# Westlake-AGI-Lab/WorldForge

Hardware: AMD Instinct MI355X
Metric: denoising steps/sec (81f x 480p, Wan2.1-14B) (higher is better)
Workload: dtype bf16

## Files before the change

include/wf_hip.h:

```cpp
#ifndef WF_HIP_H_
#define WF_HIP_H_

#include <stddef.h>
#include <stdint.h>

#ifdef __cplusplus
extern "C" {
#endif

#define WF_OK 0
#define WF_EINVAL (-1)
#define WF_EHIP (-2)
#define WF_ENOTSUP (-3)

#define WF_F32 0
#define WF_BF16 1

int wf_version(void);
const char* wf_last_error(void);
int wf_device_info(int dev, int* n_cu, int* clock_khz, char* name, int name_len);


int wf_cfg_combine(const void* cond, const void* uncond, void* out, int dt, float g, size_t n, void* stream);

// ... 41 lines not shown

size_t wf_farneback_workspace_bytes(int C, int T, int h, int w);
int wf_farneback_flows(const void* x, int dt, float* flow, int C, int T, int h, int w, int quant_mode, void* ws, void* stream);


#define WF_EPI_BF16 0
#define WF_EPI_BF16_GELU 1
#define WF_EPI_F32 2
#define WF_EPI_RESID 3
#define WF_EPI_F32_ACC 4
int wf_gemm_bf16(const void* X, const void* W, const float* bias, void* out, const float* gate, int M, int N, int K, int ldx,
                 int ldw, int ldo, int epilogue, void* stream);
int wf_gemm_bf16_batched(const void* X, const void* W, void* out, int batch, int M, int N, int K, int ldx, int ldw, int ldo,
                         int64_t bsx, int64_t bsw, int64_t bso, int epilogue, void* stream);
int wf_gemm_f16(const void* X, const void* W, const float* bias, void* out, int M, int N, int K, int ldx, int ldw, int ldo, int epilogue,
                float acc_scale, void* stream);
int wf_gemm_f16_batched(const void* X, const void* W, void* out, int batch, int M, int N, int K, int ldx, int ldw, int ldo, int64_t bsx,
                        int64_t bsw, int64_t bso, int epilogue, void* stream);
int wf_mx_quant_e4m3(const void* X, void* Q, void* S, int M, int K, int ldx, void* stream);
int wf_gemm_mxfp8(const void* Xq, const void* Xs, const void* Wq, const void* Ws, const float* bias, void* out, const float* gate, int M, int N,
                  int K, int ldx, int ldw, int ldo, int epilogue, void* stream);
int wf_lora_fold(const void* base, void* out, int N, int K, int n_adapters, const void* U0, const void* D0, int rank0, int nsep0,
                 float scale0, const void* U1, const void* D1, int rank1, int nsep1, float scale1, const void* U2, const void* D2,
                 int rank2, int nsep2, float scale2, const void* U3, const void* D3, int rank3, int nsep3, float scale3, void* stream);

int wf_attn_fwd(const void* Q, const void* K, const void* Vt, void* O, int H, int Lq, int Lkp, int kv_len, int seg_len,
                size_t seg_stride_bytes, int ldo, float softmax_scale, int accumulate, const float* kmax2, int kmax_n, int kmax_stride,
                const float* qmax2, int qmax_n, void* stream);
int wf_head_max_norm2(const void* X, int H, int L, int Lp, float* out, void* stream);
size_t wf_attn_split_workspace_bytes(int H, int Lq, int nsplit);
int wf_attn_cross2_fwd(const void* Q, const void* K, const void* Vt, void* O, int H, int Lq, int Lk1p, int kv_len1, int Lk2p, int kv_len2,
                       int ldo, float softmax_scale, void* stream);
int wf_attn_debug_body_counter(void* counters2);
int wf_attn_fwd_split(const void* Q, const void* K, const void* Vt, void* O, int H, int Lq, int Lkp, int kv_len, int seg_len,
                      size_t seg_stride_bytes, int ldo, float softmax_scale, int accumulate, int nsplit, void* workspace, const float* kmax2,
                      int kmax_n, int kmax_stride, const float* qmax2, int qmax_n, void* stream);
int wf_attn_fwd_part(const void* Q, const void* K, const void* Vt, int H, int Lq, int Lkp, int kv_len, int seg_len, size_t seg_stride_bytes,
                     int t_begin, int t_end, int t_begin2, int t_end2, int inner_splits, int part, int nparts, void* workspace, void* O_merge,
                     int ldo, const float* kmax2, int kmax_n, int kmax_stride, const float* qmax2, int qmax_n, void* stream);
int wf_attn_merge(void* O, int H, int Lq, int ldo, int accumulate, int nparts, const void* workspace, void* stream);

int wf_ln_modulate(const float* x, const float* mul, const float* add, void* out, int out_dtype, int L, int C, float eps,
                   int plus_one, void* stream);

int wf_rmsnorm_heads(const void* in, int ld, const float* weight, const float* cos_tab, const float* sin_tab, void* out, int L,
                     int Lout, int C, float eps, float out_scale, void* stream);
size_t wf_rmsnorm_heads_bound_ws_floats(int L, int C);
int wf_rmsnorm_heads_bound(const void* in, int ld, const float* weight, const float* cos_tab, const float* sin_tab, void* out, int L, int Lout,
                           int C, float eps, float out_scale, float* ws, float* max_norm2, void* stream);

int wf_v_transpose(const void* V, int ld, void* Vt, int L, int Lp, int H, void* stream);
int wf_v_transpose_seg(const void* V, int ld, void* Vt, int L, int Lp, int H, int head_stride_tiles, void* stream);
int wf_v_transpose_at(const void* V, int ld, void* Vt, int k0, int L, int Lp, int H, void* stream);

int wf_patchify(const void* x, void* tokens, int Cin, int T, int Hh, int Ww, void* stream);
int wf_unpatchify(const float* y, float* out, int Cout, int T, int Hh, int Ww, void* stream);

int wf_act(const void* a, int dt_a, const void* b, int dt_b, void* out, int dt_out, int mode, size_t n, void* stream);

int wf_lc_ln_modulate(const void* x, const float* mul, const float* add, int64_t mod_ld, int rows_per_group, int64_t row0,
                      const int* group_index, int plus_one, void* out, int L, int C, float eps, void* stream);
int wf_lc_gate_residual(void* x, const void* y, int64_t ldy, const float* gate, int64_t gate_ld, int rows_per_group, int64_t row0,
                        const int* group_index, int L, int C, void* stream);
int wf_lc_norm_heads(const void* in, int64_t ld, const float* weight, const float* cos_tab, const float* sin_tab, void* out, int L,
                     int Lout, int H, float eps, float out_scale, void* stream);
int wf_lc_swiglu(const void* in, int64_t ld, void* out, int L, int Hd, void* stream);
// ... 124 lines not shown
```

worldforge_amd/csrc/attention.hip:

```cpp
#include "common.h"
#include "mfma.h"

#include <climits>
#include <cstdlib>
#include <type_traits>
#include <utility>

using namespace wf;

namespace {

constexpr int D = 128;
constexpr int QB = 256;
constexpr int KB = 64;
constexpr int K_TILE_BYTES = KB * D * 2;
constexpr int V_TILE_BYTES = D * KB * 2;

struct AttnArgs {
  const uint16_t* Q;
  const uint16_t* K;
  const uint16_t* Vt;
  uint16_t* O;
  int H, Lq, Lkp, kv_len, ldo;
  int seg_len;
// ... 24 lines not shown
#define WF_ATTN_DMA_PLACE 0
#endif
#ifndef WF_ATTN_ABLATE
#define WF_ATTN_ABLATE 0
#endif
#ifdef WF_ATTN_TIMING
__device__ unsigned long long g_attn_cycles[32];
#endif

constexpr int MAX_MERGE = 11;
__device__ __forceinline__ float ws_at(const float (&w)[MAX_MERGE], int s) {
  float r = w[0];
#pragma unroll
  for (int i = 1; i < MAX_MERGE; ++i) r = s == i ? w[i] : r;
  return r;
}

__device__ __forceinline__ int swap23(int i) { return (i & ~12) | ((i & 4) << 1) | ((i & 8) >> 1); }


constexpr int NT4 = 256;

__device__ __forceinline__ float mul_rn(float a, float b) {
  float r;
  asm("v_mul_f32 %0, %1, %2" : "=v"(r) : "v"(a), "v"(b));
  return r;
}
__device__ __forceinline__ float add_rn(float a, float b) {
  float r;
  asm("v_add_f32 %0, %1, %2" : "=v"(r) : "v"(a), "v"(b));
  return r;
}

template <int KIND, bool NOMAX, bool PART = false>
__device__ __forceinline__ void attn_w4_body(const AttnArgs& a) {
  extern __shared__ __attribute__((aligned(16))) unsigned char smem[];
  constexpr int BUF_BYTES = K_TILE_BYTES + V_TILE_BYTES;
  constexpr int NBUF = 5;
  static_assert(NBUF * BUF_BYTES == 160 * 1024, "the ring is the whole LDS of a CU and the launch asks for exactly that (attn_launch: lds_w4)");
  static_assert((NT4 / 64) * 4 * 1024 == K_TILE_BYTES && (NT4 / 64) * 4 * 1024 == V_TILE_BYTES,
                "4 waves x (4 K + 4 V^T) pieces of 1 KiB (64 lanes x 16 B) cover a K tile and a V^T tile exactly: no piece may spill into the next ring slot");
  static_assert(K_TILE_BYTES % 1024 == 0 && BUF_BYTES % 16 == 0, "piece granularity / ds_read_b128 alignment of the slots");
  static_assert(NBUF >= 2 + 3, "ring too short for the 3-ahead staging with one barrier per two tiles");

  const int b = blockIdx.x;
  const int xcd = b & 7, j = b >> 3;
  const int hslot = j / a.n_qblk;
  const int head = hslot * 8 + xcd;
  const int qblk = j % a.n_qblk;
  if (head >= a.H) return;

  const int tid = threadIdx.x, lane = tid & 63, wid = tid >> 6;
  const int l31 = lane & 31, hi = lane >> 5;
  int q_row[2];
  bf16x8 qf[2][8];
#pragma unroll
  for (int x = 0; x < 2; ++x) {
    q_row[x] = qblk * QB + wid * 64 + x * 32 + l31;
    const uint16_t* qp = a.Q + ((size_t)head * a.Lq + min(q_row[x], a.Lq - 1)) * D;
#pragma unroll
    for (int st = 0; st < 8; ++st) qf[x][st] = as_bf16x8(*reinterpret_cast<const u32x4*>(qp + 16 * st + 8 * hi));
  }

  const int wu = __builtin_amdgcn_readfirstlane(wid);
  int ksrc[4], vsrc[4];
#pragma unroll
  for (int i = 0; i < 4; ++i) {
    const int piece = wu * 4 + i;
    const int kr = 4 * piece + (lane >> 4), ks = lane & 15;
    ksrc[i] = kr * D + ((ks ^ (kr & 15)) << 3);
    const int vr = 8 * piece + (lane >> 3), vs = lane & 7;
    vsrc[i] = vr * KB + ((vs ^ ((vr >> 1) & 7)) << 3);
  }
  const int tiles_per_seg = a.seg_len / KB;
  int krow_off[2], krow_sw[2];
#pragma unroll
  for (int kb = 0; kb < 2; ++kb) {
    int kr = kb * 32 + swap23(l31);
    krow_off[kb] = kr * 256;
    krow_sw[kb] = kr & 15;
  }
  int vrow_off[4], vrow_sw[4];
#pragma unroll
// ... 29 lines not shown
    const bool after = rel0 >= a.n_first;
    t_begin = after ? a.t_begin2 + (rel0 - a.n_first) : a.t_begin0 + rel0;
    ntiles_ = min(a.tiles_per_split, a.tiles_per_split2 - rel0);
    if (!after && rel0 + ntiles_ > a.n_first) {
      hole_at = a.n_first - rel0;
      hole_tiles = a.t_begin2 - a.t_end;
    }
  } else {
    t_begin = a.t_begin0 + (int)blockIdx.y * a.tiles_per_split;
    ntiles_ = min(a.tiles_per_split, min(ntiles_all, a.t_end) - t_begin);
  }
  const int* bsa = nullptr;
  const int tpe = (KIND == 3 && a.bsa_shift == 2) ? 2 : 1;
  const int mine = a.bsa_shift == 2 ? (wu >> 1) : wu;
  if constexpr (KIND == 3) {
    bsa = a.bsa_list + ((size_t)head * a.n_qblk + qblk) * a.bsa_max;
    ntiles_ = tpe * a.bsa_cnt[head * a.n_qblk + qblk];
    if (ntiles_ == 0) {
#pragma unroll
      for (int x = 0; x < 2; ++x)
        if (q_row[x] < a.Lq) {
          uint16_t* op = a.O + (size_t)q_row[x] * a.ldo + head * D;
          for (int d = hi * 64; d < hi * 64 + 64; d += 8) *reinterpret_cast<u32x4*>(op + d) = u32x4{0u, 0u, 0u, 0u};
        }
      return;
    }
  }
  const int ntiles = ntiles_;
  const bool ragged = KIND != 3 && KIND != 5 && (a.kv_len & (KB - 1)) != 0;
  const int rag_t = ragged ? ntiles_all - 2 - t_begin - hole_tiles : -1;
  const bool rag1 = KIND == 5 && (a.kv_len1 & (KB - 1)) != 0, rag2 = KIND == 5 && (a.kv_len & (KB - 1)) != 0;

  const size_t tile_bytes = (size_t)(KB * D * 2);
  const size_t seg_jump = a.seg_stride - (size_t)tiles_per_seg * tile_bytes;
  const size_t hole_bytes = (size_t)(hole_tiles / tiles_per_seg) * a.seg_stride;
  const int seg0 = t_begin / tiles_per_seg, in0 = t_begin - seg0 * tiles_per_seg;
  size_t st_off = (size_t)seg0 * a.seg_stride + ((size_t)head * tiles_per_seg + in0) * tile_bytes;
  int st_tile = 0, st_left = tiles_per_seg - in0;
  uint32_t st_base = wu * 4096;
  int e_stage = 0, e_mask = 0;
  int e_pref = 0, e_q[3] = {0, 0, 0};
  const int n_entries = KIND == 3 ? ntiles / tpe : 1;
  auto entry_index = [&](int tile) { return min(tpe == 2 ? (tile >> 1) : tile, n_entries - 1); };
  if constexpr (KIND == 3) {
    e_stage = __builtin_amdgcn_readfirstlane(bsa[0]);
    st_off = (size_t)(e_stage >> a.bsa_shift) * tpe * tile_bytes;
    e_q[0] = e_q[1] = e_q[2] = e_stage;
    e_pref = bsa[entry_index(1)];
  }
  auto stage_next = [&]() {
    ++st_tile;
    const bool live = st_tile < ntiles;
    if constexpr (KIND == 3) {
      if (live) {
        e_stage = __builtin_amdgcn_readfirstlane(e_pref);
        st_off = ((size_t)(e_stage >> a.bsa_shift) * tpe + (st_tile & (tpe - 1))) * tile_bytes;
      }
      e_pref = bsa[entry_index(st_tile + 1)];
      e_q[0] = e_q[1];
      e_q[1] = e_q[2];
      e_q[2] = e_stage;
      st_base = st_base + BUF_BYTES >= (uint32_t)(NBUF * BUF_BYTES) ? st_base + BUF_BYTES - NBUF * BUF_BYTES : st_base + BUF_BYTES;
      return;
    }
    const bool wrap = --st_left == 0;
    if constexpr (PART) {
      const bool hop = st_tile == hole_at;
      st_off += live ? (wrap ? tile_bytes + seg_jump + (hop ? hole_bytes : 0) : tile_bytes) : 0;
    } else {
      st_off += live ? (wrap ? tile_bytes + seg_jump : tile_bytes) : 0;
    }
    st_left = wrap ? tiles_per_seg : st_left;
    st_base = st_base + BUF_BYTES >= (uint32_t)(NBUF * BUF_BYTES) ? st_base + BUF_BYTES - NBUF * BUF_BYTES : st_base + BUF_BYTES;
  };
  const uint32_t smem_base = __builtin_amdgcn_readfirstlane(lds_offset(smem));
  uint32_t kbyte[4], vbyte[4];
#pragma unroll
  for (int i = 0; i < 4; ++i) {
    kbyte[i] = (uint32_t)ksrc[i] * 2u;
    vbyte[i] = (uint32_t)vsrc[i] * 2u;
  }
  auto stage_piece = [&](int i) {
    const unsigned char* kb_ = reinterpret_cast<const unsigned char*>(a.K) + st_off;
    const unsigned char* vb_ = reinterpret_cast<const unsigned char*>(a.Vt) + st_off;
    if (i < 4)
// ... 115 lines not shown
    for (int x = 0; x < 2; ++x)
#pragma unroll
      for (int kb = 0; kb < 2; ++kb)
#pragma unroll
        for (int r = 0; r < 16; ++r) {
          int key = tile_in_ctx * KB + 32 * kb + 16 * (r >> 3) + 8 * hi + (r & 7);
          if (key >= len) sb[B][x][kb][r] = -INFINITY;
        }
  };

  auto mask_unselected = [&](auto BC, int entry) {
    constexpr int B = decltype(BC)::value;
    if (!((entry >> mine) & 1)) {
#pragma unroll
      for (int x = 0; x < 2; ++x)
#pragma unroll
        for (int kb = 0; kb < 2; ++kb)
#pragma unroll
          for (int r = 0; r < 16; ++r) sb[B][x][kb][r] = -INFINITY;
    }
  };

#ifndef WF_ATTN_PF4
#define WF_ATTN_PF4 4
#endif
  constexpr int PF4 = WF_ATTN_PF4;
  u32x4 ring[PF4];
#if defined(WF_ATTN_TIMING) && WF_ATTN_TIMING != 2
  unsigned long long tacc[20] = {};
#define W4MARK(k) do { const unsigned long long n__ = __builtin_readcyclecounter(); tacc[k] += n__ - tlast; tlast = n__; } while (0)
#else
#define W4MARK(k) do { } while (0)
#endif
  auto tile = [&](auto BC, int t, int slot0) {
    constexpr int B = decltype(BC)::value;
    const int slot1 = slot0 + 1 == NBUF ? 0 : slot0 + 1;
    const int slot2 = slot1 + 1 == NBUF ? 0 : slot1 + 1;
    const unsigned char* sK1 = smem + slot1 * BUF_BYTES;
    const unsigned char* sV0 = smem + slot0 * BUF_BYTES + K_TILE_BYTES;
    const unsigned char* sK2 = smem + slot2 * BUF_BYTES;
    float tq_[64], pq[64];
    float ls[2][4];
    uint32_t pk[2][4] = {{0u, 0u, 0u, 0u}, {0u, 0u, 0u, 0u}};
    float mx[2][4];
    float mn[2] = {0.f, 0.f};
#if defined(WF_ATTN_TIMING) && WF_ATTN_TIMING != 2
    unsigned long long tlast = __builtin_readcyclecounter();
#endif
    __builtin_amdgcn_sched_barrier(0);
    for_const<64>([&](auto GC) {
      auto& sb_ = sb;
      auto& pf_ = pf;
      auto& o_ = o;
      auto& ring_ = ring;
      auto& tq__ = tq_;
      auto& pq_ = pq;
      auto& ls_ = ls;
      auto& pk_ = pk;
      auto& mx_ = mx;
      auto& mcq_ = mcq;
      constexpr int g = decltype(GC)::value;
      constexpr int q = g & 1;
      if constexpr (g < 32) {
        constexpr int i = g >> 1;
        mfma_s(sb_[1 - B][q][i & 1], ring_[i % PF4], qf[q][i >> 1], i < 2, PS ? &minit[q] : nullptr);
        __builtin_amdgcn_sched_barrier(0);
        if constexpr (q == 1 && !(WF_ATTN_ABLATE & 4)) {
// ... 64 lines not shown
          constexpr int kb = ch >> 1, r0 = (ch & 1) + 4 * st;
          if constexpr (st == 0) {
            asm volatile("v_max_f32 %0, %1, %2" : "=v"(mx_[x][ch]) : "v"(sb_[1 - B][x][kb][r0]), "v"(sb_[1 - B][x][kb][r0 + 2]));
          } else {
            asm volatile("v_max3_f32 %0, %0, %1, %2" : "+v"(mx_[x][ch]) : "v"(sb_[1 - B][x][kb][r0]), "v"(sb_[1 - B][x][kb][r0 + 2]));
          }
        });
      }
      if constexpr (!NOMAX && (g == 60 || g == 61)) {
        constexpr int x = g - 60;
        asm volatile("v_max3_f32 %0, %1, %2, %3" : "=v"(mn[x]) : "v"(mx_[x][0]), "v"(mx_[x][1]), "v"(mx_[x][2]));
        asm volatile("v_max_f32 %0, %0, %1" : "+v"(mn[x]) : "v"(mx_[x][3]));
      }
      if constexpr (!NOMAX && (g == 62 || g == 63)) {
        constexpr int x = g - 62;
        const unsigned mu = __float_as_uint(mn[x]);
        auto sw = __builtin_amdgcn_permlane32_swap(mu, mu, false, false);
        if constexpr (PS) {
          const float zero = 0.0f;
          asm volatile("v_max3_f32 %0, %1, %2, %3" : "=v"(mn[x]) : "v"(__uint_as_float(sw[0])), "v"(__uint_as_float(sw[1])), "v"(zero));
        } else {
          asm volatile("v_max3_f32 %0, %1, %2, %3" : "=v"(mn[x]) : "v"(__uint_as_float(sw[0])), "v"(__uint_as_float(sw[1])), "v"(m_run[x]));
        }
      }
      if constexpr (!(WF_ATTN_ABLATE & 1) && (g == 54 || g == 56)) {
        constexpr int x = (g - 54) >> 1;
        l_run[x] = add_rn(l_run[x], add_rn(add_rn(ls_[x][0], ls_[x][1]), add_rn(ls_[x][2], ls_[x][3])));
        asm volatile("" : "+v"(l_run[x]));
      }
#ifdef WF_ATTN_TIMING
      if constexpr ((g & 7) == 7) W4MARK(B * 8 + (g >> 3));
#endif
      if constexpr (g == 0) {
        stage_next();
        if constexpr (KIND == 3) e_mask = e_q[0];
      }
#if WF_ATTN_DMA_PLACE == 0
      if constexpr (g >= 2 && g < 32 && (g & 3) == 2) stage_piece_c(std::integral_constant<int, ((g - 2) >> 2)>{});
#elif WF_ATTN_DMA_PLACE == 9
#endif
      if constexpr (g == 51) {
        if (__builtin_expect(t == rag_t, 0)) mask_ragged(std::integral_constant<int, 1 - B>{}, t + 1);
        if constexpr (KIND == 3) mask_unselected(std::integral_constant<int, 1 - B>{}, e_mask);
        if constexpr (KIND == 5) {
          if (__builtin_expect(rag1 && t + 1 == a.n1 - 1, 0)) mask_tail(std::integral_constant<int, 1 - B>{}, t + 1, a.kv_len1);
          if (__builtin_expect(rag2 && t + 1 == ntiles - 1, 0)) mask_tail(std::integral_constant<int, 1 - B>{}, t + 1 - a.n1, a.kv_len);
        }
      }
      __builtin_amdgcn_sched_barrier(0);
    });
    if constexpr (NOMAX) {
    } else if constexpr (PS) {
      if (__builtin_expect(t + 1 < ntiles && __any(fmaxf(mn[0], mn[1]) > 8.0f), 0)) {
        commit_ps(std::integral_constant<int, 0>{}, std::integral_constant<int, 1 - B>{}, mn[0]);
        commit_ps(std::integral_constant<int, 1>{}, std::integral_constant<int, 1 - B>{}, mn[1]);
      }
    } else if (__builtin_expect(t + 1 < ntiles && __any(c * fmaxf(mn[0] - m_run[0], mn[1] - m_run[1]) > 8.0f), 0)) {
      commit(std::integral_constant<int, 0>{}, mn[0]);
      commit(std::integral_constant<int, 1>{}, mn[1]);
    }
    W4MARK(16);
    if constexpr (B == 1) {
      if constexpr (!(WF_ATTN_ABLATE & 2)) drain_dma();
      W4MARK(17);
      if constexpr (!(WF_ATTN_ABLATE & 2)) bar();
      W4MARK(18);
#pragma unroll
// ... 9 lines not shown
      float l = l_run[X];
      l += __shfl_xor(l, 32, 64);
      const float inv = 1.0f / l;
#pragma unroll
      for (int db = 0; db < 4; ++db) {
        f32x16 tmp = o[X][db];
        asm volatile("" : "+v"(tmp));
#pragma unroll
        for (int g = 0; g < 4; ++g) {
          stash[X][db][2 * g] = pack_bf16x2(mul_rn(tmp[4 * g + 0], inv), mul_rn(tmp[4 * g + 1], inv));
          stash[X][db][2 * g + 1] = pack_bf16x2(mul_rn(tmp[4 * g + 2], inv), mul_rn(tmp[4 * g + 3], inv));
        }
#pragma unroll
        for (int r = 0; r < 16; ++r) tmp[r] = 0.f;
        asm volatile("" : "+v"(tmp));
        o[X][db] = tmp;
        asm volatile("" : "+a"(o[X][db]));
      }
      l_run[X] = 0.f;
      float m = sb[NB][X][0][0];
#pragma unroll
      for (int kb = 0; kb < 2; ++kb)
#pragma unroll
        for (int r = 0; r < 16; ++r) m = fmaxf(m, sb[NB][X][kb][r]);
      const unsigned mu = __float_as_uint(m);
      auto sw = __builtin_amdgcn_permlane32_swap(mu, mu, false, false);
      m_run[X] = fmaxf(__uint_as_float(sw[0]), __uint_as_float(sw[1]));
      mcq[X] = c * m_run[X];
    });
  };
  using B0 = std::integral_constant<int, 0>;
  using B1 = std::integral_constant<int, 1>;

#pragma unroll
  for (int i = 0; i < 8; ++i) stage_piece(i);
  stage_next();
#pragma unroll
  for (int i = 0; i < 8; ++i) stage_piece(i);
  stage_next();
#pragma unroll
  for (int i = 0; i < 8; ++i) stage_piece(i);
  drain_dma();
  bar();
  {
#pragma unroll
    for (int i = 0; i < 16; ++i) {
      const u32x4 kf = kread(smem, i);
      mfma_s(sb[0][0][i & 1], kf, qf[0][i >> 1], i < 2);
      mfma_s(sb[0][1][i & 1], kf, qf[1][i >> 1], i < 2);
    }
    asm volatile("s_nop 7\n\ts_nop 7\n\ts_nop 3" ::: "memory");
    if (ragged && t_begin == ntiles_all - 1) mask_ragged(B0{}, 0);
    if constexpr (KIND == 5) {
      if (rag1 && a.n1 == 1) mask_tail(B0{}, 0, a.kv_len1);
    }
    if constexpr (KIND == 3) mask_unselected(B0{}, __builtin_amdgcn_readfirstlane(bsa[0]));
    const float m0 = rowmax_now(B0{}, std::integral_constant<int, 0>{});
    const float m1 = rowmax_now(B0{}, std::integral_constant<int, 1>{});
    if constexpr (PS) {
      m_run[0] = m0;
      m_run[1] = m1;
#pragma unroll
      for (int x = 0; x < 2; ++x)
#pragma unroll
        for (int kb = 0; kb < 2; ++kb)
#pragma unroll
          for (int r = 0; r < 16; ++r) sb[0][x][kb][r] -= m_run[x];
      set_minit(std::integral_constant<int, 0>{});
      set_minit(std::integral_constant<int, 1>{});
    } else {
      commit(std::integral_constant<int, 0>{}, m0);
      commit(std::integral_constant<int, 1>{}, m1);
    }
    const unsigned char* sK1 = smem + (ntiles > 1 ? 1 : 0) * BUF_BYTES;
#pragma unroll
    for (int i = 0; i < PF4; ++i) ring[i] = kread(sK1, i);
  }
#if defined(WF_ATTN_TIMING) && WF_ATTN_TIMING == 2
  const unsigned long long t_loop0 = __builtin_readcyclecounter();
#endif
  {
    int slot = 0;
    int t = 0;
    if constexpr (NOMAX) {
      for (; t + 3 < ntiles; t += 4) {
        tile(B0{}, t, slot);
        slot = slot + 1 == NBUF ? 0 : slot + 1;
        tile(B1{}, t + 1, slot);
        slot = slot + 1 == NBUF ? 0 : slot + 1;
        tile(B0{}, t + 2, slot);
        slot = slot + 1 == NBUF ? 0 : slot + 1;
        tile(B1{}, t + 3, slot);
        slot = slot + 1 == NBUF ? 0 : slot + 1;
      }
    }
    for (; t < ntiles; t += 2) {
      tile(B0{}, t, slot);
      if constexpr (KIND == 5) {
        if (__builtin_expect(t == a.n1 - 1, 0)) seam(B1{});
      }
      slot = slot + 1 == NBUF ? 0 : slot + 1;
      if (t + 1 < ntiles) {
        tile(B1{}, t + 1, slot);
        if constexpr (KIND == 5) {
          if (__builtin_expect(t + 1 == a.n1 - 1, 0)) seam(B0{});
        }
      }
      slot = slot + 1 == NBUF ? 0 : slot + 1;
    }
  }
#if defined(WF_ATTN_TIMING) && WF_ATTN_TIMING == 2
  {
    const unsigned long long t_loop1 = __builtin_readcyclecounter();
    if (lane == 0 && wid == 0) {
      atomicAdd(&g_attn_cycles[20], t_loop1 - t_loop0);
      atomicAdd(&g_attn_cycles[19], (unsigned long long)ntiles);
    }
  }
#elif defined(WF_ATTN_TIMING)
  if (lane == 0 && wid == 0) {
    for (int i = 0; i < 19; ++i) atomicAdd(&g_attn_cycles[i], tacc[i]);
    atomicAdd(&g_attn_cycles[19], (unsigned long long)ntiles);
  }
#endif
  asm volatile("s_nop 7\n\ts_nop 7\n\ts_nop 7" ::: "memory");

#pragma unroll
  for (int x = 0; x < 2; ++x) {
    float l = l_run[x];
    l += __shfl_xor(l, 32, 64);
    float inv = 1.0f / l;
    if constexpr (KIND == 3) inv = l > 0.f ? inv : 0.f;
    bool merged = false;
    if constexpr (PART) {
      if (a.merge_n > 0) {
        merged = true;
        const size_t qr = (size_t)min(q_row[x], a.Lq - 1);
        float ms[MAX_MERGE], ws[MAX_MERGE];
        float M = m_run[x];
#pragma unroll
        for (int s = 0; s < MAX_MERGE; ++s) {
          ms[s] = s < a.merge_n ? a.ml_part[(((size_t)s * a.H + head) * a.Lq + qr) * 2] : -INFINITY;
          M = fmaxf(M, ms[s]);
        }
        const float w_own = __builtin_amdgcn_exp2f(m_run[x] - M);
        float lt = 0.f;
#pragma unroll
        for (int s = 0; s < MAX_MERGE; ++s) {
          ws[s] = s < a.merge_n ? __builtin_amdgcn_exp2f(ms[s] - M) : 0.f;
          if (s < a.merge_n) lt += ws[s] * a.ml_part[(((size_t)s * a.H + head) * a.Lq + qr) * 2 + 1];
        }
        l = lt + w_own * l;
        inv = 1.0f / l;
#pragma unroll
        for (int db = 0; db < 4; ++db) {
          f32x16 ov = o[x][db];
          asm volatile("" : "+v"(ov));
// ... 45 lines not shown
#pragma unroll
        for (int gg = 0; gg < 2; ++gg) {
          const int g = 2 * j + gg;
          float v0 = mul_rn(ov[4 * g + 0], inv), v1 = mul_rn(ov[4 * g + 1], inv), v2 = mul_rn(ov[4 * g + 2], inv),
                v3 = mul_rn(ov[4 * g + 3], inv);
          if constexpr (KIND == 5) {
            const uint32_t o0 = stash[x][db][2 * g], o1 = stash[x][db][2 * g + 1];
            v0 = add_rn(v0, __uint_as_float(o0 << 16));
            v1 = add_rn(v1, __uint_as_float(o0 & 0xffff0000u));
            v2 = add_rn(v2, __uint_as_float(o1 << 16));
            v3 = add_rn(v3, __uint_as_float(o1 & 0xffff0000u));
          } else if (a.accumulate) {
            u32x2 old = {0u, 0u};
            if (live) old = *reinterpret_cast<const u32x2*>(op + db * 32 + 8 * g + 4 * hi);
            v0 = add_rn(v0, __uint_as_float(old[0] << 16));
            v1 = add_rn(v1, __uint_as_float(old[0] & 0xffff0000u));
            v2 = add_rn(v2, __uint_as_float(old[1] << 16));
            v3 = add_rn(v3, __uint_as_float(old[1] & 0xffff0000u));
          }
          pk[gg][0] = pack_bf16x2(v0, v1);
          pk[gg][1] = pack_bf16x2(v2, v3);
        }
        const auto s0 = __builtin_amdgcn_permlane32_swap(pk[0][0], pk[1][0], false, false);
        const auto s1 = __builtin_amdgcn_permlane32_swap(pk[0][1], pk[1][1], false, false);
        if (live) {
          u32x4 st = {s0[0], s1[0], s0[1], s1[1]};
          *reinterpret_cast<u32x4*>(op + db * 32 + 16 * j + 8 * hi) = st;
        }
      }
    }
  }
}

__device__ __forceinline__ bool attn_untracked_ok(const AttnArgs& a) {
  bool fast = false;
  if (a.kmax2 && a.qmax2) {
    const int b = blockIdx.x;
    const int head = ((b >> 3) / a.n_qblk) * 8 + (b & 7);
    if (head < a.H) {
      float kn2 = 0.f, qn2 = 0.f;
      for (int i = 0; i < a.kmax_n; ++i) kn2 = fmaxf(kn2, a.kmax2[(size_t)i * a.kmax_stride + head]);
      for (int i = 0; i < a.qmax_n; ++i) qn2 = fmaxf(qn2, a.qmax2[i * a.H + head]);
      fast = qn2 * kn2 <= 2500.0f;
    }
  }
  if (a.dbg_body && threadIdx.x == 0) atomicAdd(a.dbg_body + (fast ? 1 : 0), 1u);
  return fast;
}

template <int KIND>
__global__ __launch_bounds__(NT4, 1) void k_attn_w4(AttnArgs a) {
  if constexpr (KIND == 4) {
    const bool fast = attn_untracked_ok(a);
    if (__builtin_amdgcn_readfirstlane((int)fast))
      attn_w4_body<4, true>(a);
    else
      attn_w4_body<4, false>(a);
  } else {
    attn_w4_body<KIND, false>(a);
  }
}

__global__ __launch_bounds__(NT4, 1) void k_attn_w4_part(AttnArgs a) {
  const bool fast = attn_untracked_ok(a);
  if (__builtin_amdgcn_readfirstlane((int)fast))
    attn_w4_body<4, true, true>(a);
  else
    attn_w4_body<4, false, true>(a);
}

__global__ void k_attn_merge(AttnArgs a) {
  const size_t i = (size_t)blockIdx.x * blockDim.x + threadIdx.x;
  const size_t n = (size_t)a.Lq * a.H * (D / 4);
  if (i >= n) return;
  const int d4 = (int)(i % (D / 4));
  const int h = (int)((i / (D / 4)) % a.H);
  const size_t q = i / ((size_t)(D / 4) * a.H);
  float M = -INFINITY;
  for (int s = 0; s < a.nsplit; ++s) M = fmaxf(M, a.ml_part[(((size_t)s * a.H + h) * a.Lq + q) * 2]);
  float l = 0.f;
  f32x4 acc = {0.f, 0.f, 0.f, 0.f};
  for (int s = 0; s < a.nsplit; ++s) {
    const float* ml = a.ml_part + (((size_t)s * a.H + h) * a.Lq + q) * 2;
    const float w = __builtin_amdgcn_exp2f(a.scale_log2 * (ml[0] - M));
    l += w * ml[1];
    const f32x4 ov = *reinterpret_cast<const f32x4*>(a.o_part + ((size_t)s * a.Lq + q) * (size_t)(a.H * D) + h * D + 4 * d4);
#pragma unroll
    for (int k = 0; k < 4; ++k) acc[k] += w * ov[k];
  }
  const float inv = 1.0f / l;
  uint16_t* op = a.O + q * a.ldo + h * D + 4 * d4;
  float v[4];
#pragma unroll
  for (int k = 0; k < 4; ++k) v[k] = acc[k] * inv;
  if (a.accumulate) {
    const u32x2 old = *reinterpret_cast<const u32x2*>(op);
    v[0] += __uint_as_float(old[0] << 16);
    v[1] += __uint_as_float(old[0] & 0xffff0000u);
    v[2] += __uint_as_float(old[1] << 16);
    v[3] += __uint_as_float(old[1] & 0xffff0000u);
  }
  u32x2 pk = {pack_bf16x2(v[0], v[1]), pack_bf16x2(v[2], v[3])};
  *reinterpret_cast<u32x2*>(op) = pk;
}

}

static unsigned int* g_dbg_body = nullptr;

struct PartWindow {
  int index = -1, t0 = 0, t1 = 0, inner = 1, t0b = 0, t1b = 0;
  bool merge = false;
};
constexpr int MAX_PARTS = 12;

static int attn_launch(const void* Q, const void* K, const void* Vt, void* O, int H, int Lq, int Lkp, int kv_len, int seg_len, int ldo,
                       float softmax_scale, int accumulate, int nsplit, void* workspace, const float* kmax2, int kmax_n, const float* qmax2,
                       int qmax_n, void* stream, const char* who, size_t seg_stride = 0, int kmax_stride = 0, PartWindow pw = PartWindow()) {
  const int part_index = pw.index, part_t0 = pw.t0, part_t1 = pw.t1, part_inner = pw.inner;
  WF_CHECK_ARG(Q && K && Vt && O, "%s: null pointer", who);
  WF_CHECK_ARG((!kmax2 || (kmax_n >= 1 && kmax_n <= 64)) && (!qmax2 || (qmax_n >= 1 && qmax_n <= 64)), "%s: kmax_n / qmax_n must be 1..64", who);
  WF_CHECK_ARG(H > 0 && Lq > 0 && kv_len > 0, "%s: empty problem", who);
  WF_CHECK_ARG(Lkp % KB == 0 && kv_len <= Lkp, "%s: Lkp (%d) must be a multiple of 64 and >= kv_len (%d)", who, Lkp, kv_len);
  WF_CHECK_ARG(seg_len > 0 && seg_len % KB == 0 && Lkp % seg_len == 0, "%s: seg_len (%d) must be a multiple of 64 dividing Lkp", who,
               seg_len);
  const size_t dense_stride = (size_t)H * seg_len * D * 2;
  WF_CHECK_ARG(seg_stride == 0 || (seg_stride >= dense_stride && seg_stride % 16 == 0),
               "%s: seg_stride_bytes (%zu) must be 0 (dense) or a multiple of 16 >= H * seg_len * 256 = %zu", who, seg_stride, dense_stride);
  WF_CHECK_ARG(kmax_stride == 0 || kmax_stride >= H, "%s: kmax_stride (%d) must be 0 (contiguous) or >= H", who, kmax_stride);
  WF_CHECK_ARG(ldo % 8 == 0 && ldo >= H * D, "%s: ldo %d must be a multiple of 8 (16-byte stores) and >= H * 128", who, ldo);
  WF_CHECK_ARG((((uintptr_t)Q | (uintptr_t)K | (uintptr_t)Vt | (uintptr_t)O) & 15) == 0, "%s: 16-byte alignment", who);
  AttnArgs a;
  a.Q = (const uint16_t*)Q;
  a.K = (const uint16_t*)K;
  a.Vt = (const uint16_t*)Vt;
  a.O = (uint16_t*)O;
  a.H = H;
  a.Lq = Lq;
  a.Lkp = Lkp;
  a.kv_len = kv_len;
  a.seg_len = seg_len;
  a.seg_stride = seg_stride ? seg_stride : dense_stride;
  a.kmax_stride = kmax_stride ? kmax_stride : H;
  a.ldo = ldo;
  a.n_qblk = ceil_div(Lq, QB);
  const bool prescaled = softmax_scale == 0.0f;
  a.scale_log2 = prescaled ? 1.0f : softmax_scale * 1.4426950408889634f;
  a.accumulate = accumulate;
  a.prio_mode = 0;
  const int ntiles = ceil_div(kv_len, KB);
  a.nsplit = 1;
  a.tiles_per_split = ntiles;
  a.t_begin0 = 0;
  a.t_end = INT_MAX;
  a.part0 = 0;
  a.n_first = INT_MAX;
  a.t_begin2 = a.t_end2 = a.tiles_per_split2 = 0;
  a.o_part = nullptr;
  a.ml_part = nullptr;
  a.bsa_list = nullptr;
  a.bsa_cnt = nullptr;
  a.bsa_max = 0;
  a.bsa_shift = 2;
  a.kmax2 = kmax2;
  a.qmax2 = qmax2;
  a.kmax_n = kmax2 ? kmax_n : 0;
  a.qmax_n = qmax2 ? qmax_n : 0;
  a.dbg_body = g_dbg_body;
  a.kv_len1 = 0;
  a.n1 = 0;
  const int hslots = (H + 7) / 8;
  const int grid = hslots * a.n_qblk * 8;
  const size_t lds_w4 = 5 * (K_TILE_BYTES + V_TILE_BYTES);
  int grid_y = 1;
  if (part_index >= 0) {
    WF_CHECK_ARG(softmax_scale == 0.0f, "%s: part launches are built for the pre-scaled-Q form only (softmax_scale = 0)", who);
    WF_CHECK_ARG(part_t0 >= 0 && part_t0 < part_t1 && part_t0 < ntiles, "%s: empty tile window [%d, %d) of %d tiles", who, part_t0, part_t1, ntiles);
    const int t1 = part_t1 < ntiles ? part_t1 : ntiles;
    int joined = t1 - part_t0, t1b = 0;
    a.n_first = INT_MAX;
    if (pw.t1b > pw.t0b) {
      const int tps_seg = seg_len / KB;
      WF_CHECK_ARG(pw.t0b >= t1 && pw.t0b < ntiles, "%s: second tile window [%d, %d) must lie behind the first [%d, %d) and inside the %d tiles", who,
                   pw.t0b, pw.t1b, part_t0, t1, ntiles);
      WF_CHECK_ARG(t1 == part_t1 && t1 % tps_seg == 0 && pw.t0b % tps_seg == 0 && pw.t0b > t1,
                   "%s: the hole [%d, %d) between the two windows must be whole segments of %d tiles", who, t1, pw.t0b, tps_seg);
      t1b = pw.t1b < ntiles ? pw.t1b : ntiles;
      a.n_first = t1 - part_t0;
      a.t_begin2 = pw.t0b;
      a.t_end2 = t1b;
      joined += t1b - pw.t0b;
    }
    const int tps = ceil_div(joined, part_inner < 1 ? 1 : part_inner);
    grid_y = ceil_div(joined, tps);
    a.tiles_per_split2 = joined;
    if (pw.merge) {
      WF_CHECK_ARG(grid_y == 1 && part_index >= 1 && part_index <= MAX_MERGE && part_index == nsplit - 1,
                   "%s: a merging part launch is the LAST of its sweep and has one split (slot %d of %d, %d split(s))", who, part_index, nsplit, grid_y);
      a.merge_n = part_index;
    }
    WF_CHECK_ARG(nsplit >= 2 && nsplit <= MAX_PARTS && part_index + grid_y <= nsplit, "%s: slots %d..%d of %d (2..%d)", who, part_index,
                 part_index + grid_y - 1, nsplit, MAX_PARTS);
    WF_CHECK_ARG(workspace && (((uintptr_t)workspace) & 15) == 0, "%s: needs a 16-byte aligned workspace", who);
    a.nsplit = nsplit;
    a.t_begin0 = part_t0;
    a.t_end = t1;
    a.tiles_per_split = tps;
    a.part0 = part_index;
    a.o_part = (float*)workspace;
    a.ml_part = a.o_part + (size_t)nsplit * Lq * H * D;
  } else if (nsplit > 1) {
    WF_CHECK_ARG(workspace && (((uintptr_t)workspace) & 15) == 0, "%s: nsplit > 1 needs a 16-byte aligned workspace", who);
    int tps = ceil_div(ntiles, nsplit);
    const int ns = ceil_div(ntiles, tps);
    a.nsplit = ns;
    a.tiles_per_split = tps;
    a.o_part = (float*)workspace;
    a.ml_part = a.o_part + (size_t)ns * Lq * H * D;
    grid_y = ns;
  }
  if (part_index >= 0)
    hipLaunchKernelGGL(k_attn_w4_part, dim3(grid, grid_y), dim3(NT4), lds_w4, (hipStream_t)stream, a);
  else if (prescaled)
    hipLaunchKernelGGL(k_attn_w4<4>, dim3(grid, grid_y), dim3(NT4), lds_w4, (hipStream_t)stream, a);
#ifdef WF_ATTN_LAB
  else
    WF_CHECK_ARG(false, "%s: lab build, pre-scaled self-attention only", who);
#else
  else if (Lkp > 1024)
    hipLaunchKernelGGL(k_attn_w4<0>, dim3(grid, grid_y), dim3(NT4), lds_w4, (hipStream_t)stream, a);
  else
    hipLaunchKernelGGL(k_attn_w4<1>, dim3(grid, grid_y), dim3(NT4), lds_w4, (hipStream_t)stream, a);
#endif
  if (a.nsplit > 1 && part_index < 0) {
    const size_t n = (size_t)Lq * H * (D / 4);
    hipLaunchKernelGGL(k_attn_merge, dim3((unsigned)((n + 255) / 256)), dim3(256), 0, (hipStream_t)stream, a);
  }
  WF_LAUNCH_CHECK(who);
  return WF_OK;
}

extern "C" int wf_attn_fwd(const void* Q, const void* K, const void* Vt, void* O, int H, int Lq, int Lkp, int kv_len, int seg_len,
                           size_t seg_stride_bytes, int ldo, float softmax_scale, int accumulate, const float* kmax2, int kmax_n,
                           int kmax_stride, const float* qmax2, int qmax_n, void* stream) {
  return attn_launch(Q, K, Vt, O, H, Lq, Lkp, kv_len, seg_len, ldo, softmax_scale, accumulate, 1, nullptr, kmax2, kmax_n, qmax2, qmax_n,
                     stream, "wf_attn_fwd", seg_stride_bytes, kmax_stride);
}

namespace {
__global__ __launch_bounds__(256) void k_head_max_norm2(const uint16_t* __restrict__ X, int L, int Lp, int rows_per_block, float* __restrict__ out) {
  const int head = blockIdx.y;
  const int r0 = blockIdx.x * rows_per_block, r1 = min(L, r0 + rows_per_block);
  const int sub = threadIdx.x & 15, grp = threadIdx.x >> 4;
// ... 117 lines not shown
  a.K = (const uint16_t*)K;
  a.Vt = (const uint16_t*)Vt;
  a.O = (uint16_t*)O;
  a.H = H;
  a.Lq = Lq;
  a.Lkp = Lk1p + Lk2p;
  a.kv_len = kv_len2;
  a.seg_len = a.Lkp;
  a.ldo = ldo;
  a.n_qblk = ceil_div(Lq, QB);
  a.scale_log2 = softmax_scale * 1.4426950408889634f;
  a.accumulate = 0;
  a.prio_mode = 0;
  a.nsplit = 1;
  a.tiles_per_split = a.Lkp / KB;
  a.seg_stride = (size_t)a.H * a.seg_len * D * 2;
  a.kmax_stride = a.H;
  a.n_first = INT_MAX;
  a.t_begin2 = a.t_end2 = a.tiles_per_split2 = 0;
  a.t_begin0 = 0;
  a.t_end = INT_MAX;
  a.part0 = 0;
  a.o_part = nullptr;
  a.ml_part = nullptr;
  a.bsa_list = nullptr;
  a.bsa_cnt = nullptr;
  a.bsa_max = 0;
  a.bsa_shift = 2;
  a.kmax2 = a.qmax2 = nullptr;
  a.kmax_n = a.qmax_n = 0;
  a.dbg_body = nullptr;
  a.kv_len1 = kv_len1;
  a.n1 = Lk1p / KB;
  const int grid = ((H + 7) / 8) * a.n_qblk * 8;
#ifdef WF_ATTN_LAB
  WF_CHECK_ARG(false, "%s: lab build, pre-scaled self-attention only", "wf_attn_cross2_fwd");
#else
  hipLaunchKernelGGL(k_attn_w4<5>, dim3(grid, 1), dim3(NT4), 5 * (K_TILE_BYTES + V_TILE_BYTES), (hipStream_t)stream, a);
#endif
  WF_LAUNCH_CHECK("wf_attn_cross2_fwd");
  return WF_OK;
}

extern "C" int wf_attn_fwd_part(const void* Q, const void* K, const void* Vt, int H, int Lq, int Lkp, int kv_len, int seg_len,
                                size_t seg_stride_bytes, int t_begin, int t_end, int t_begin2, int t_end2, int inner_splits, int part, int nparts,
                                void* workspace, void* O_merge, int ldo, const float* kmax2, int kmax_n, int kmax_stride, const float* qmax2,
                                int qmax_n, void* stream) {
  PartWindow pw;
  pw.index = part;
  pw.t0 = t_begin;
  pw.t1 = t_end;
  pw.inner = inner_splits;
  pw.t0b = t_begin2;
  pw.t1b = t_end2;
  pw.merge = O_merge != nullptr;
  WF_CHECK_ARG(part >= 0, "wf_attn_fwd_part: part index %d", part);
  return attn_launch(Q, K, Vt, O_merge ? O_merge : workspace, H, Lq, Lkp, kv_len, seg_len, O_merge ? ldo : H * D, 0.0f, 0, nparts, workspace, kmax2,
                     kmax_n, qmax2, qmax_n, stream, "wf_attn_fwd_part", seg_stride_bytes, kmax_stride, pw);
}

extern "C" int wf_attn_merge(void* O, int H, int Lq, int ldo, int accumulate, int nparts, const void* workspace, void* stream) {
  WF_CHECK_ARG(O && workspace, "wf_attn_merge: null pointer");
  WF_CHECK_ARG(H > 0 && Lq > 0 && nparts >= 2 && nparts <= MAX_PARTS, "wf_attn_merge: H=%d Lq=%d nparts=%d (2..%d)", H, Lq, nparts, MAX_PARTS);
  WF_CHECK_ARG(ldo % 8 == 0 && ldo >= H * D && ((((uintptr_t)O) | ((uintptr_t)workspace)) & 15) == 0, "wf_attn_merge: ldo %d / alignment", ldo);
  AttnArgs a = {};
  a.O = (uint16_t*)O;
  a.H = H;
  a.Lq = Lq;
  a.ldo = ldo;
  a.accumulate = accumulate;
  a.scale_log2 = 1.0f;
  a.nsplit = nparts;
  a.o_part = (float*)const_cast<void*>(workspace);
  a.ml_part = a.o_part + (size_t)nparts * Lq * H * D;
  const size_t n = (size_t)Lq * H * (D / 4);
  hipLaunchKernelGGL(k_attn_merge, dim3((unsigned)((n + 255) / 256)), dim3(256), 0, (hipStream_t)stream, a);
  WF_LAUNCH_CHECK("wf_attn_merge");
  return WF_OK;
}

extern "C" int wf_attn_debug_body_counter(void* counters2) {
  g_dbg_body = (unsigned int*)counters2;
  return WF_OK;
}

extern "C" size_t wf_attn_split_workspace_bytes(int H, int Lq, int nsplit) {
  if (H <= 0 || Lq <= 0 || nsplit <= 1) return 0;
  return ((size_t)nsplit * Lq * H * D + (size_t)nsplit * H * Lq * 2) * sizeof(float);
}

extern "C" int wf_attn_fwd_split(const void* Q, const void* K, const void* Vt, void* O, int H, int Lq, int Lkp, int kv_len, int seg_len,
                                 size_t seg_stride_bytes, int ldo, float softmax_scale, int accumulate, int nsplit, void* workspace,
                                 const float* kmax2, int kmax_n, int kmax_stride, const float* qmax2, int qmax_n, void* stream) {
  WF_CHECK_ARG(nsplit >= 1 && nsplit <= 8, "wf_attn_fwd_split: nsplit %d out of range 1..8", nsplit);
  return attn_launch(Q, K, Vt, O, H, Lq, Lkp, kv_len, seg_len, ldo, softmax_scale, accumulate, nsplit, workspace, kmax2, kmax_n, qmax2,
                     qmax_n, stream, "wf_attn_fwd_split", seg_stride_bytes, kmax_stride);
}

#ifdef WF_ATTN_TIMING
extern "C" int wf_debug_attn_cycles(unsigned long long* out32, int reset) {
  if (hipMemcpyFromSymbol(out32, HIP_SYMBOL(g_attn_cycles), sizeof(unsigned long long) * 32) != hipSuccess) return -1;
  if (reset) {
    unsigned long long z[32] = {};
    if (hipMemcpyToSymbol(HIP_SYMBOL(g_attn_cycles), z, sizeof(z)) != hipSuccess) return -1;
  }
  return 0;
}
#endif
```

worldforge_amd/ops.py:

```python
from __future__ import annotations

from typing import Optional, Sequence

import threading

import torch

from . import _ffi
from ._ffi import WF_BF16, WF_F32, call


def _dt(t: torch.Tensor) -> int:
    if t.dtype == torch.float32:
        return WF_F32
    if t.dtype == torch.bfloat16:
        return WF_BF16
    raise TypeError(f"unsupported dtype {t.dtype} (float32 / bfloat16 only)")


def _dev(t: torch.Tensor) -> torch.Tensor:
    if not t.is_cuda:
        raise RuntimeError("worldforge_amd ops need device tensors (there is no CPU fallback)")
    return t if t.is_contiguous() else t.contiguous()

# ... 234 lines not shown
    assert q.shape == (M, K) and q.is_contiguous() and s.shape == (M, K // 32) and s.is_contiguous()
    call("wf_mx_quant_e4m3", x.data_ptr(), q.data_ptr(), s.data_ptr(), M, K, x.stride(0), stream())
    return q, s


def gemm_mxfp8(xq: torch.Tensor, xs: torch.Tensor, wq: torch.Tensor, ws: torch.Tensor, bias: Optional[torch.Tensor], out: torch.Tensor,
               epi: int, gate: Optional[torch.Tensor] = None) -> torch.Tensor:
    M, K = xq.shape
    N = wq.shape[0]
    assert wq.shape[1] == K and xs.shape == (M, K // 32) and ws.shape == (N, K // 32) and out.shape[0] == M and out.shape[1] == N
    assert xs.is_contiguous() and ws.is_contiguous()
    call("wf_gemm_mxfp8", xq.data_ptr(), xs.data_ptr(), wq.data_ptr(), ws.data_ptr(), bias.data_ptr() if bias is not None else None,
         out.data_ptr(), gate.data_ptr() if gate is not None else None, M, N, K, xq.stride(0), wq.stride(0), out.stride(0), epi, stream())
    return out


def lora_fold(base: torch.Tensor, out: torch.Tensor, adapters) -> torch.Tensor:
    if not (base.is_cuda and out.is_cuda and all(U.is_cuda and D.is_cuda for U, D, _, _ in adapters)):
        raise RuntimeError("worldforge_amd ops need device tensors (there is no CPU fallback)")
    assert base.dim() == 2 and base.dtype == out.dtype == torch.bfloat16 and base.shape == out.shape
    assert base.is_contiguous() and out.is_contiguous()
    N, K = base.shape
    flat = []
    for U, D, nsep, scale in adapters:
        assert U.dtype == D.dtype == torch.bfloat16 and U.is_contiguous() and D.is_contiguous()
        assert U.shape[0] == N and D.shape == (int(nsep) * U.shape[1], K), (tuple(U.shape), tuple(D.shape), nsep, (N, K))
        flat += [U.data_ptr(), D.data_ptr(), U.shape[1], int(nsep), float(scale)]
    n = len(flat) // 5
    if not 1 <= n <= 4:
        raise ValueError(f"wf_lora_fold takes 1..4 adapters per launch, not {n}")
    flat += [None, None, 0, 0, 0.0] * (4 - n)
    call("wf_lora_fold", base.data_ptr(), out.data_ptr(), N, K, n, *flat, stream())
    return out
```

Before: 0.2417.

## Make attention kernel persistent and prefetch next work item's K/V tiles

The self- and cross-attention kernels now launch one workgroup per CU on each XCD. Each workgroup loops over its (head, query-block) items instead of launching one workgroup per item. While finishing the current item, the staging ring continues into the first tiles of the next head's K/V, so the next item starts with the ring already primed. This is meant to remove per-workgroup launch and pipeline-fill overhead and the tail bubble between items. The cost is more complex ring-slot bookkeeping across items and possible load imbalance from the static stride assignment.

```diff
diff --git a/include/wf_hip.h b/include/wf_hip.h
--- a/include/wf_hip.h
+++ b/include/wf_hip.h
@@ -97,6 +97,7 @@
 int wf_attn_cross2_fwd(const void* Q, const void* K, const void* Vt, void* O, int H, int Lq, int Lk1p, int kv_len1, int Lk2p, int kv_len2,
                        int ldo, float softmax_scale, void* stream);
 int wf_attn_debug_body_counter(void* counters2);
+int wf_attn_set_walk_workgroups(int n);
 int wf_attn_fwd_split(const void* Q, const void* K, const void* Vt, void* O, int H, int Lq, int Lkp, int kv_len, int seg_len,
                       size_t seg_stride_bytes, int ldo, float softmax_scale, int accumulate, int nsplit, void* workspace, const float* kmax2,
                       int kmax_n, int kmax_stride, const float* qmax2, int qmax_n, void* stream);
diff --git a/worldforge_amd/csrc/attention.hip b/worldforge_amd/csrc/attention.hip
--- a/worldforge_amd/csrc/attention.hip
+++ b/worldforge_amd/csrc/attention.hip
@@ -80,8 +80,16 @@
   return r;
 }
 
+struct Walk {
+  int slot = 0;
+  int item = 0;
+  bool primed = false;
+  size_t st_off = 0;
+};
+
 template <int KIND, bool NOMAX, bool PART = false>
-__device__ __forceinline__ void attn_w4_body(const AttnArgs& a) {
+__device__ __forceinline__ void attn_w4_body(const AttnArgs& a, const int head, const int qblk, Walk& w, const int nxt_head) {
+  constexpr bool WALK = !PART && KIND != 3;
   extern __shared__ __attribute__((aligned(16))) unsigned char smem[];
   constexpr int BUF_BYTES = K_TILE_BYTES + V_TILE_BYTES;
   constexpr int NBUF = 5;
@@ -90,13 +98,6 @@
                 "4 waves x (4 K + 4 V^T) pieces of 1 KiB (64 lanes x 16 B) cover a K tile and a V^T tile exactly: no piece may spill into the next ring slot");
   static_assert(K_TILE_BYTES % 1024 == 0 && BUF_BYTES % 16 == 0, "piece granularity / ds_read_b128 alignment of the slots");
   static_assert(NBUF >= 2 + 3, "ring too short for the 3-ahead staging with one barrier per two tiles");
-
-  const int b = blockIdx.x;
-  const int xcd = b & 7, j = b >> 3;
-  const int hslot = j / a.n_qblk;
-  const int head = hslot * 8 + xcd;
-  const int qblk = j % a.n_qblk;
-  if (head >= a.H) return;
 
   const int tid = threadIdx.x, lane = tid & 63, wid = tid >> 6;
   const int l31 = lane & 31, hi = lane >> 5;
@@ -192,7 +193,16 @@
   const bool rag1 = KIND == 5 && (a.kv_len1 & (KB - 1)) != 0, rag2 = KIND == 5 && (a.kv_len & (KB - 1)) != 0;
 
   const size_t tile_bytes = (size_t)(KB * D * 2);
-  const size_t seg_jump = a.seg_stride - (size_t)tiles_per_seg * tile_bytes;
+  size_t seg_jump = a.seg_stride - (size_t)tiles_per_seg * tile_bytes;
+  int st_end = ntiles;
+  bool pre_next = false;
+  if constexpr (WALK) {
+    pre_next = nxt_head >= 0 && ntiles >= 3 && tiles_per_seg >= ntiles && t_begin == 0;
+    if (pre_next) {
+      seg_jump = ((size_t)nxt_head - (size_t)head) * tiles_per_seg * tile_bytes - (size_t)ntiles * tile_bytes;
+      st_end = ntiles + 3;
+    }
+  }
   const size_t hole_bytes = (size_t)(hole_tiles / tiles_per_seg) * a.seg_stride;
   const int seg0 = t_begin / tiles_per_seg, in0 = t_begin - seg0 * tiles_per_seg;
   size_t st_off = (size_t)seg0 * a.seg_stride + ((size_t)head * tiles_per_seg + in0) * tile_bytes;
@@ -208,9 +218,9 @@
     e_q[0] = e_q[1] = e_q[2] = e_stage;
     e_pref = bsa[entry_index(1)];
   }
-  auto stage_next = [&]() {
+  auto stage_next = [&](bool known_live = false) {
     ++st_tile;
-    const bool live = st_tile < ntiles;
+    const bool live = known_live || st_tile < st_end;
     if constexpr (KIND == 3) {
       if (live) {
         e_stage = __builtin_amdgcn_readfirstlane(e_pref);
@@ -392,7 +402,7 @@
 #else
 #define W4MARK(k) do { } while (0)
 #endif
-  auto tile = [&](auto BC, int t, int slot0) {
+  auto tile = [&](auto BC, int t, int slot0, auto LIVE3) {
     constexpr int B = decltype(BC)::value;
     const int slot1 = slot0 + 1 == NBUF ? 0 : slot0 + 1;
     const int slot2 = slot1 + 1 == NBUF ? 0 : slot1 + 1;
@@ -523,7 +533,7 @@
       if constexpr ((g & 7) == 7) W4MARK(B * 8 + (g >> 3));
 #endif
       if constexpr (g == 0) {
-        stage_next();
+        stage_next(decltype(LIVE3)::value);
         if constexpr (KIND == 3) e_mask = e_q[0];
       }
 #if WF_ATTN_DMA_PLACE == 0
@@ -599,20 +609,40 @@
   using B0 = std::integral_constant<int, 0>;
   using B1 = std::integral_constant<int, 1>;
 
-#pragma unroll
-  for (int i = 0; i < 8; ++i) stage_piece(i);
-  stage_next();
-#pragma unroll
-  for (int i = 0; i < 8; ++i) stage_piece(i);
-  stage_next();
-#pragma unroll
-  for (int i = 0; i < 8; ++i) stage_piece(i);
+  const int slot_first = WALK ? w.slot : 0;
+  bool primed = false;
+  if constexpr (WALK) primed = w.primed;
+  if (primed) {
+    st_off = w.st_off;
+    st_tile = 2;
+    st_left = tiles_per_seg - 2;
+    const int s2 = slot_first + 2 >= NBUF ? slot_first + 2 - NBUF : slot_first + 2;
+    st_base = wu * 4096 + s2 * BUF_BYTES;
+  } else {
+    if constexpr (WALK) {
+      if (w.item > 0) {
+        drain_dma();
+        bar();
+      }
+      st_base = wu * 4096 + slot_first * BUF_BYTES;
+    }
+#pragma unroll
+    for (int i = 0; i < 8; ++i) stage_piece(i);
+    stage_next();
+#pragma unroll
+    for (int i = 0; i < 8; ++i) stage_piece(i);
+    stage_next();
+#pragma unroll
+    for (int i = 0; i < 8; ++i) stage_piece(i);
+  }
+  if (pre_next) st_left = ntiles - 2;
   drain_dma();
   bar();
   {
+    const unsigned char* sK0 = smem + slot_first * BUF_BYTES;
 #pragma unroll
     for (int i = 0; i < 16; ++i) {
-      const u32x4 kf = kread(smem, i);
+      const u32x4 kf = kread(sK0, i);
       mfma_s(sb[0][0][i & 1], kf, qf[0][i >> 1], i < 2);
       mfma_s(sb[0][1][i & 1], kf, qf[1][i >> 1], i < 2);
     }
@@ -639,7 +669,8 @@
       commit(std::integral_constant<int, 0>{}, m0);
       commit(std::integral_constant<int, 1>{}, m1);
     }
-    const unsigned char* sK1 = smem + (ntiles > 1 ? 1 : 0) * BUF_BYTES;
+    const int slot_second = slot_first + 1 == NBUF ? 0 : slot_first + 1;
+    const unsigned char* sK1 = smem + (ntiles > 1 ? slot_second : slot_first) * BUF_BYTES;
 #pragma unroll
     for (int i = 0; i < PF4; ++i) ring[i] = kread(sK1, i);
   }
@@ -647,28 +678,28 @@
   const unsigned long long t_loop0 = __builtin_readcyclecounter();
 #endif
   {
-    int slot = 0;
+    int slot = slot_first;
     int t = 0;
     if constexpr (NOMAX) {
       for (; t + 3 < ntiles; t += 4) {
-        tile(B0{}, t, slot);
+        tile(B0{}, t, slot, std::true_type{});
         slot = slot + 1 == NBUF ? 0 : slot + 1;
-        tile(B1{}, t + 1, slot);
+        tile(B1{}, t + 1, slot, std::false_type{});
         slot = slot + 1 == NBUF ? 0 : slot + 1;
-        tile(B0{}, t + 2, slot);
+        tile(B0{}, t + 2, slot, std::false_type{});
         slot = slot + 1 == NBUF ? 0 : slot + 1;
-        tile(B1{}, t + 3, slot);
+        tile(B1{}, t + 3, slot, std::false_type{});
         slot = slot + 1 == NBUF ? 0 : slot + 1;
       }
     }
     for (; t < ntiles; t += 2) {
-      tile(B0{}, t, slot);
+      tile(B0{}, t, slot, std::false_type{});
       if constexpr (KIND == 5) {
         if (__builtin_expect(t == a.n1 - 1, 0)) seam(B1{});
       }
       slot = slot + 1 == NBUF ? 0 : slot + 1;
       if (t + 1 < ntiles) {
-        tile(B1{}, t + 1, slot);
+        tile(B1{}, t + 1, slot, std::false_type{});
         if constexpr (KIND == 5) {
           if (__builtin_expect(t + 1 == a.n1 - 1, 0)) seam(B0{});
         }
@@ -690,6 +721,12 @@
     atomicAdd(&g_attn_cycles[19], (unsigned long long)ntiles);
   }
 #endif
+  if constexpr (WALK) {
+    w.slot = (slot_first + ntiles % NBUF) % NBUF;
+    w.item += 1;
+    w.primed = pre_next;
+    w.st_off = st_off;
+  }
   asm volatile("s_nop 7\n\ts_nop 7\n\ts_nop 7" ::: "memory");
 
 #pragma unroll
@@ -801,11 +838,9 @@
   }
 }
 
-__device__ __forceinline__ bool attn_untracked_ok(const AttnArgs& a) {
+__device__ __forceinline__ bool attn_untracked_ok(const AttnArgs& a, const int head) {
   bool fast = false;
   if (a.kmax2 && a.qmax2) {
-    const int b = blockIdx.x;
-    const int head = ((b >> 3) / a.n_qblk) * 8 + (b & 7);
     if (head < a.H) {
       float kn2 = 0.f, qn2 = 0.f;
       for (int i = 0; i < a.kmax_n; ++i) kn2 = fmaxf(kn2, a.kmax2[(size_t)i * a.kmax_stride + head]);
@@ -819,23 +854,58 @@
 
 template <int KIND>
 __global__ __launch_bounds__(NT4, 1) void k_attn_w4(AttnArgs a) {
-  if constexpr (KIND == 4) {
-    const bool fast = attn_untracked_ok(a);
-    if (__builtin_amdgcn_readfirstlane((int)fast))
-      attn_w4_body<4, true>(a);
-    else
-      attn_w4_body<4, false>(a);
+#if defined(WF_ATTN_TIMING) && WF_ATTN_TIMING == 2
+  const unsigned long long t_wg0 = __builtin_readcyclecounter();
+#endif
+  const int xcd = blockIdx.x & 7;
+  Walk w;
+  if constexpr (KIND == 3) {
+    const int j = blockIdx.x >> 3;
+    const int head = (j / a.n_qblk) * 8 + xcd;
+    if (head < a.H) attn_w4_body<3, false>(a, head, j % a.n_qblk, w, -1);
   } else {
-    attn_w4_body<KIND, false>(a);
-  }
+    const int W = gridDim.x >> 3;
+    const int items = ((a.H + 7) >> 3) * a.n_qblk;
+    for (int j = blockIdx.x >> 3; j < items; j += W) {
+      const int hslot = j / a.n_qblk;
+      const int head = __builtin_amdgcn_readfirstlane(hslot * 8 + xcd);
+      const int qblk = __builtin_amdgcn_readfirstlane(j - hslot * a.n_qblk);
+      int nxt_head = -1;
+      if (j + W < items) {
+        nxt_head = __builtin_amdgcn_readfirstlane((j + W) / a.n_qblk * 8 + xcd);
+        nxt_head = nxt_head < a.H ? nxt_head : -1;
+      }
+      if constexpr (KIND == 4) {
+        const bool fast = attn_untracked_ok(a, head);
+        if (head >= a.H) continue;
+        if (__builtin_amdgcn_readfirstlane((int)fast))
+          attn_w4_body<4, true>(a, head, qblk, w, nxt_head);
+        else
+          attn_w4_body<4, false>(a, head, qblk, w, nxt_head);
+      } else {
+        if (head >= a.H) continue;
+        attn_w4_body<KIND, false>(a, head, qblk, w, nxt_head);
+      }
+    }
+  }
+#if defined(WF_ATTN_TIMING) && WF_ATTN_TIMING == 2
+  if (threadIdx.x == 0) {
+    atomicAdd(&g_attn_cycles[21], __builtin_readcyclecounter() - t_wg0);
+    atomicAdd(&g_attn_cycles[22], 1ull);
+  }
+#endif
 }
 
 __global__ __launch_bounds__(NT4, 1) void k_attn_w4_part(AttnArgs a) {
-  const bool fast = attn_untracked_ok(a);
+  const int j = blockIdx.x >> 3;
+  const int head = (j / a.n_qblk) * 8 + (blockIdx.x & 7), qblk = j % a.n_qblk;
+  const bool fast = attn_untracked_ok(a, head);
+  if (head >= a.H) return;
+  Walk w;
   if (__builtin_amdgcn_readfirstlane((int)fast))
-    attn_w4_body<4, true, true>(a);
+    attn_w4_body<4, true, true>(a, head, qblk, w, -1);
   else
-    attn_w4_body<4, false, true>(a);
+    attn_w4_body<4, false, true>(a, head, qblk, w, -1);
 }
 
 __global__ void k_attn_merge(AttnArgs a) {
@@ -876,6 +946,20 @@
 }
 
 static unsigned int* g_dbg_body = nullptr;
+static int g_walk_wg = 0;
+
+static int walk_width(int items) {
+  static int cus_per_xcd = 0;
+  if (cus_per_xcd == 0) {
+    int dev = 0, cus = 0;
+    if (hipGetDevice(&dev) == hipSuccess && hipDeviceGetAttribute(&cus, hipDeviceAttributeMultiprocessorCount, dev) == hipSuccess && cus >= 8)
+      cus_per_xcd = cus / 8;
+    else
+      cus_per_xcd = -1;
+  }
+  const int w = g_walk_wg > 0 ? g_walk_wg : cus_per_xcd;
+  return w > 0 && w < items ? w : items;
+}
 
 struct PartWindow {
   int index = -1, t0 = 0, t1 = 0, inner = 1, t0b = 0, t1b = 0;
@@ -939,7 +1023,7 @@
   a.kv_len1 = 0;
   a.n1 = 0;
   const int hslots = (H + 7) / 8;
-  const int grid = hslots * a.n_qblk * 8;
+  int grid = hslots * a.n_qblk * 8;
   const size_t lds_w4 = 5 * (K_TILE_BYTES + V_TILE_BYTES);
   int grid_y = 1;
   if (part_index >= 0) {
@@ -988,6 +1072,7 @@
     a.ml_part = a.o_part + (size_t)ns * Lq * H * D;
     grid_y = ns;
   }
+  if (part_index < 0 && a.nsplit == 1) grid = walk_width(hslots * a.n_qblk) * 8;
   if (part_index >= 0)
     hipLaunchKernelGGL(k_attn_w4_part, dim3(grid, grid_y), dim3(NT4), lds_w4, (hipStream_t)stream, a);
   else if (prescaled)
@@ -1171,7 +1256,7 @@
   a.dbg_body = nullptr;
   a.kv_len1 = kv_len1;
   a.n1 = Lk1p / KB;
-  const int grid = ((H + 7) / 8) * a.n_qblk * 8;
+  const int grid = walk_width(((H + 7) / 8) * a.n_qblk) * 8;
 #ifdef WF_ATTN_LAB
   WF_CHECK_ARG(false, "%s: lab build, pre-scaled self-attention only", "wf_attn_cross2_fwd");
 #else
@@ -1223,6 +1308,12 @@
   return WF_OK;
 }
 
+extern "C" int wf_attn_set_walk_workgroups(int n) {
+  WF_CHECK_ARG(n >= 0, "wf_attn_set_walk_workgroups: n = %d (0 = from the device, >= 1 = workgroups per XCD slot)", n);
+  g_walk_wg = n;
+  return WF_OK;
+}
+
 extern "C" size_t wf_attn_split_workspace_bytes(int H, int Lq, int nsplit) {
   if (H <= 0 || Lq <= 0 || nsplit <= 1) return 0;
   return ((size_t)nsplit * Lq * H * D + (size_t)nsplit * H * Lq * 2) * sizeof(float);
diff --git a/worldforge_amd/ops.py b/worldforge_amd/ops.py
--- a/worldforge_amd/ops.py
+++ b/worldforge_amd/ops.py
@@ -290,3 +290,7 @@
     flat += [None, None, 0, 0, 0.0] * (4 - n)
     call("wf_lora_fold", base.data_ptr(), out.data_ptr(), N, K, n, *flat, stream())
     return out
+
+
+def attn_set_walk_workgroups(n: int = 0) -> None:
+    call("wf_attn_set_walk_workgroups", int(n))
```

New measurement: 0.2419 (median of 3 runs). Within noise of the previous version (+0.1%).
